# HKUST-Aerial-Robotics/VINS-Mobile

Hardware: AMD Instinct MI355X
Metric: VIO frames/sec (KLT+window solve), 640x480/150 feats/W=10 (higher is better)
Workload: dtype f64 (solve) / u8+i32+f32 (KLT)

## Files before the change

### vins-mobile_amd/abi.py

```python
import ctypes as C
import os

import numpy as np

VIO_OK = 0
VIO_EINVAL, VIO_ENODEV, VIO_ENOMEM, VIO_ECAP, VIO_ESTATE, VIO_ETIMEOUT = -1, -2, -3, -4, -5, -6
VIO_MAX_PRIOR_BLOCKS = 96
VIO_MAX_TRACE = 64
VIO_INIT_BA_MAX_FRAMES = 32
VIO_BLOCK_POSE, VIO_BLOCK_SPEEDBIAS, VIO_BLOCK_EXPOSE = 0, 1, 2
VIO_MARGIN_OLD, VIO_MARGIN_SECOND_NEW, VIO_MARGIN_NONE = 0, 1, 2
STAGES = ["setup_imu", "setup_prior", "eval_prior", "eval_imu", "eval_proj", "scale", "schur", "rhs", "cholesky",
          "tri_solve", "quad_form", "dogleg", "cost_eval", "new2old", "marg_build", "marg_chol", "total",
          "p_zero", "p_fact", "p_gram", "p_feat", "c_potrf", "c_trsm", "imu_raw", "c_wait", "q_w", "backsolve",
          "c_ahead", "tr_vec", "m_prior", "m_imu", "m_fact", "m_gram", "d0", "d1", "d2", "d3", "d4", "d5",
          "v_gd", "v_dot", "v_step", "v_plus", "v_gmax", "v_rest", "b_init", "b_pose", "b_asp", "b_band", "b_gn",
          "e_head", "e_copy", "e_h0dx", "e_tail", "x0", "x1", "x2", "x3", "s0", "s1", "s2", "s3"]

_dp = C.POINTER(C.c_double)
_ip = C.POINTER(C.c_int32)


class VioConfig(C.Structure):
    _fields_ = [
        ("window_size", C.c_int32), ("max_features", C.c_int32), ("max_factors", C.c_int32),
        ("max_iterations", C.c_int32), ("image_rows", C.c_int32), ("image_cols", C.c_int32),
        ("max_corners", C.c_int32), ("min_dist", C.c_int32), ("freq", C.c_int32),
        ("lk_win", C.c_int32), ("lk_levels", C.c_int32), ("lk_max_iters", C.c_int32),
        ("lk_eps", C.c_double), ("lk_min_eig", C.c_double), ("quality_level", C.c_double),
        ("f_threshold", C.c_double), ("f_confidence", C.c_double),
        ("fx", C.c_double), ("fy", C.c_double), ("cx", C.c_double), ("cy", C.c_double),
        ("gravity", C.c_double), ("acc_n", C.c_double), ("acc_w", C.c_double),
        ("gyr_n", C.c_double), ("gyr_w", C.c_double), ("cauchy_a", C.c_double),
    ]


def hip_runtime(lib=None):
    lib = lib or load_product()
    buf, n = C.create_string_buffer(4096), C.c_int32()
    lib.vio_hip_runtime(buf, 4096, C.byref(n))
    return [p for p in buf.value.decode().split(";") if p]


def host_pool_width():
    lib = load_product()
    n = C.c_int32(0)
    return int(lib.vio_host_pool_width(C.byref(n))), int(n.value)


def default_config(**kw):
    c = VioConfig(
        window_size=10, max_features=1000, max_factors=8192, max_iterations=10,
        image_rows=640, image_cols=480, max_corners=70, min_dist=30, freq=3,
        lk_win=21, lk_levels=3, lk_max_iters=30, lk_eps=0.01, lk_min_eig=1e-4,
        quality_level=0.01, f_threshold=1.0, f_confidence=0.99,
        fx=526.600, fy=526.678, cx=243.481, cy=315.280,
        gravity=9.805, acc_n=0.5, acc_w=0.002, gyr_n=0.2, gyr_w=4.0e-5, cauchy_a=1.0)
    for k, v in kw.items():
        setattr(c, k, v)
    return c


class VioPreintegration(C.Structure):
    _fields_ = [
        ("sum_dt", C.c_double), ("delta_p", C.c_double * 3), ("delta_q", C.c_double * 4),
        ("delta_v", C.c_double * 3), ("linearized_ba", C.c_double * 3),
        ("linearized_bg", C.c_double * 3), ("jacobian", C.c_double * 225),
        ("covariance", C.c_double * 225),
    ]


PREINT_DOUBLES = C.sizeof(VioPreintegration) // 8


class VioPrior(C.Structure):
    _fields_ = [
        ("n", C.c_int32), ("n_blocks", C.c_int32),
        ("block_kind", C.c_int32 * VIO_MAX_PRIOR_BLOCKS),
        ("block_index", C.c_int32 * VIO_MAX_PRIOR_BLOCKS),
        ("block_offset", C.c_int32 * VIO_MAX_PRIOR_BLOCKS),
        ("block_x0", _dp), ("linearized_jacobians", _dp), ("linearized_residuals", _dp),
    ]


class VioWindow(C.Structure):
    _fields_ = [
        ("window_size", C.c_int32), ("n_features", C.c_int32), ("n_factors", C.c_int32),
        ("marginalization_flag", C.c_int32),
        ("pose", _dp), ("speed_bias", _dp), ("ex_pose", _dp), ("inv_depth", _dp),
        ("factor_host", _ip), ("factor_target", _ip), ("factor_feature", _ip),
        ("factor_pts_i", _dp), ("factor_pts_j", _dp),
        ("preint", C.POINTER(VioPreintegration)), ("prior", C.POINTER(VioPrior)),
        ("loop_frame", C.c_int32), ("loop_pose", _dp),
        ("use_origin_override", C.c_int32), ("origin_yaw_deg", C.c_double),
        ("origin_p", C.c_double * 3),
        ("raw_pose", _dp), ("raw_speed_bias", _dp), ("raw_inv_depth", _dp),
        ("next_prior", C.POINTER(VioPrior)),
        ("resident_prior", C.c_int32),
    ]


class VioSolveStats(C.Structure):
    _fields_ = [
        ("initial_cost", C.c_double), ("final_cost", C.c_double),
        ("iterations", C.c_int32), ("termination", C.c_int32),
        ("num_successful_steps", C.c_int32), ("num_unsuccessful_steps", C.c_int32),
        ("it_cost", C.c_double * VIO_MAX_TRACE), ("it_radius", C.c_double * VIO_MAX_TRACE),
        ("it_step_norm", C.c_double * VIO_MAX_TRACE),
        ("it_relative_decrease", C.c_double * VIO_MAX_TRACE),
        ("it_gradient_max_norm", C.c_double * VIO_MAX_TRACE),
        ("it_flags", C.c_int32 * VIO_MAX_TRACE),
    ]


class VioObs(C.Structure):
    _fields_ = [("id", C.c_int32), ("x", C.c_double), ("y", C.c_double), ("z", C.c_double)]


class VioImuMsg(C.Structure):
    _fields_ = [("header", C.c_double), ("acc", C.c_double * 3), ("gyr", C.c_double * 3)]


class VioKeyframeData(C.Structure):
    _fields_ = [("header", C.c_double), ("translation", C.c_double * 3), ("rotation", C.c_double * 4)]


class VioPnpFeature(C.Structure):
    _fields_ = [("id", C.c_int32), ("observation", C.c_double * 2), ("position", C.c_double * 3), ("track_num", C.c_int32)]


class VioVinsResult(C.Structure):
    _fields_ = [("header", C.c_double), ("Ba", C.c_double * 3), ("Bg", C.c_double * 3), ("P", C.c_double * 3),
                ("R", C.c_double * 9), ("V", C.c_double * 3)]


class VioPnpWindow(C.Structure):
    _fields_ = [("n_frames", C.c_int32), ("pose", _dp), ("speed", _dp), ("bias", _dp), ("fixed", C.POINTER(C.c_uint8)),
                ("ex_pose", _dp), ("preint", C.POINTER(VioPreintegration)), ("feat_start", _ip), ("observation", _dp),
                ("position", _dp), ("track_num", _ip)]


class VioInitFrame(C.Structure):
    _fields_ = [("header", C.c_double), ("R", C.c_double * 9), ("T", C.c_double * 3), ("is_key_frame", C.c_int32),
                ("n_samples", C.c_int32), ("dt", _dp), ("acc", _dp), ("gyr", _dp), ("acc_0", C.c_double * 3),
                ("gyr_0", C.c_double * 3)]


class VioFrameResult(C.Structure):
    _fields_ = [("action", C.c_int32), ("error", C.c_int32), ("marginalization_flag", C.c_int32),
                ("failure_reasons", C.c_int32), ("track_num", C.c_int32), ("n_features", C.c_int32),
                ("n_factors", C.c_int32), ("n_loop_factors", C.c_int32), ("stats", VioSolveStats)]


class VioInitBaProblem(C.Structure):
    _fields_ = [("frame_num", C.c_int32), ("l", C.c_int32), ("n_points", C.c_int32), ("c_rotation", _dp), ("c_translation", _dp),
                ("points", _dp), ("point_ok", C.POINTER(C.c_uint8)), ("feat_start", _ip), ("obs_frame", _ip), ("obs_xy", _dp),
                ("ok", C.c_int32)]


class VioInitSfmProblem(C.Structure):
    _fields_ = [("frame_num", C.c_int32), ("l", C.c_int32), ("n_features", C.c_int32), ("feat_start", _ip), ("obs_frame", _ip),
                ("obs_xy", _dp), ("relative_mode", C.c_int32), ("R_hint", _dp), ("n_extra", C.c_int32), ("extra_guess", _ip),
                ("extra_start", _ip), ("extra_feature", _ip), ("extra_xy", _dp), ("status", C.c_int32), ("inliers", C.c_int32),
                ("relative_R", C.c_double * 9), ("relative_T", C.c_double * 3), ("q", _dp), ("T", _dp), ("points", _dp),
                ("point_ok", C.POINTER(C.c_uint8)), ("extra_R", _dp), ("extra_T", _dp)]


(VIO_INIT_SFM_OK, VIO_INIT_SFM_FAIL_RELATIVE, VIO_INIT_SFM_FAIL_CHAIN, VIO_INIT_SFM_FAIL_BA, VIO_INIT_SFM_FAIL_PNP) = range(5)


# ... 417 lines not shown
```

### vins-mobile_amd/csrc/marg_core.h

```cpp
#pragma once

#include "solver_core.h"

namespace vio {

struct MargOut {
  int *n;
  int *kind, *index, *offset;
  double *x0;
  double *J;
  double *r;
  double *scratch;
  int ncap;
};

template <class MP>
struct MargWorkT {
  MP Am;
  int ld;
  ldsd bm;
  ldsd tol;
  ldsd ldinv;
  ldsd hff, gf, einv;
  ldsd prdx, prr;
// ... 138 lines not shown
    const double y0 = rsq_cut(b[0], tol[0]);
    const double l10 = b[1] * y0, l20 = b[3] * y0, l30 = b[6] * y0;
    const double y1 = rsq_cut(fma(-l10, l10, b[2]), tol[1]);
    const double l21 = fma(-l20, l10, b[4]) * y1, l31 = fma(-l30, l10, b[7]) * y1;
    const double y2 = rsq_cut(fma(-l21, l21, fma(-l20, l20, b[5])), tol[2]);
    const double l32 = fma(-l31, l21, fma(-l30, l20, b[8])) * y2;
    const double y3 = rsq_cut(fma(-l32, l32, fma(-l31, l31, fma(-l30, l30, b[9]))), tol[3]);
    double M[10];
    M[0] = y0;
    M[1] = -(l10 * y0) * y1, M[2] = y1;
    M[3] = -fma(l21, M[1], l20 * y0) * y2, M[4] = -(l21 * M[2]) * y2, M[5] = y2;
    M[6] = -fma(l32, M[3], fma(l31, M[1], l30 * y0)) * y3, M[7] = -fma(l32, M[4], l31 * M[2]) * y3, M[8] = -(l32 * M[5]) * y3, M[9] = y3;
    double mop = 0.0;
#pragma unroll
    for (int q = 0; q < 10; q++) mop = mi == q ? M[q] : mop;
    const v4d z = {0.0, 0.0, 0.0, 0.0};
    const v4d V = mfma_f64(mop, A[cb], z), VE = mfma_f64(mop, E[cb], z);
    const double vv = V[0], ve = VE[0];
    A = mfma_f64(-vv, vv, A);
    E = mfma_f64(-vv, ve, E);
    keep[cb] = n >= 4 * cb + kq ? vv : ve;
    const double yn = (n & 3) == 0 ? y0 : (n & 3) == 1 ? y1 : (n & 3) == 2 ? y2 : y3;
    myinv = (n >> 2) == cb ? yn : myinv;
  }
  if (n < nvalid) {
#pragma unroll
    for (int j = 0; j < 4; j++) {
      const int c = kq + 4 * j;
      if (c < nvalid) D[n * ld + c] = keep[j];
    }
    if (kq == 0) ldinv_k[n] = myinv;
  }
}

template <class MP>
VIO_DEV void dtile_trsm(MP Aik, MP Dkk, cldsd ldinv_k, int ld, int rows, int lane) {
  const int n = lane & 15, kq = lane >> 4;
  double a[4];
  dtile_load_op(Aik, n * ld + kq, a);
  const v4d b = dtile_load_acc(Dkk, kq * ld + n, ld);
  const double dg = ldinv_k[n];
  v4d acc = {0.0, 0.0, 0.0, 0.0};
#pragma unroll
  for (int s4 = 0; s4 < 4; s4++) {
    const int kk = 4 * s4 + kq;
    const double bb = kk < n ? b[s4] : (kk == n ? dg : 0.0);
    acc = mfma_f64(a[s4], bb, acc);
  }
  dtile_store_acc(Aik, kq * ld + n, ld, acc, kq, rows);
}
template <class MP>
VIO_DEV void dtile_forward_diag(MP Dkk, cldsd ldinv_k, ldsd bk, int ld, int nvalid, int lane) {
  const int c = lane & 15;
  double s = ldinv_k[c] * bk[c];
#pragma unroll
  for (int n = 0; n < 15; n++) {
    const double x = Dkk[n * ld + c], bn = bk[n];
    s = fma(n < c ? x : 0.0, n < c ? bn : 0.0, s);
  }
  __builtin_amdgcn_wave_barrier();
  if (lane < 16 && c < nvalid) bk[c] = s;
}
template <class MP>
VIO_DEV void dtile_rhs_update(MP Lik, ldsd bi, cldsd yk, int ld, int rows, int lane) {
  const int r = lane >> 2, p = lane & 3;
  auto Lr = Lik + r * ld + p;
  double s = Lr[0] * yk[p];
  s = fma(Lr[4], yk[p + 4], s);
  s = fma(Lr[8], yk[p + 8], s);
  s = fma(Lr[12], yk[p + 12], s);
  s = quad_sum_f64(s);
  if (p == 0 && r < rows) bi[r] -= s;
}
template <class MP>
VIO_DEV void dtile_update2(MP C0, MP A0, MP B0, int rows0, int cols0, MP C1, MP A1, MP B1, int rows1, int cols1, int ld, int lane) {
  const int n = lane & 15, kq = lane >> 4, op = n * ld + kq, acc = kq * ld + n;
  double a0[4], b0[4], a1[4], b1[4];
  dtile_load_op(A0, op, a0), dtile_load_op(B0, op, b0), dtile_load_op(A1, op, a1), dtile_load_op(B1, op, b1);
  v4d c0 = dtile_load_acc(C0, acc, ld), c1 = dtile_load_acc(C1, acc, ld);
#pragma unroll
  for (int s4 = 0; s4 < 4; s4++) {
    c0 = mfma_f64(-a0[s4], b0[s4], c0);
    c1 = mfma_f64(-a1[s4], b1[s4], c1);
  }
  dtile_store_acc(C0, acc, ld, c0, kq, rows0, n < cols0);
  dtile_store_acc(C1, acc, ld, c1, kq, rows1, n < cols1);
}

template <class MP>
VIO_DEV void mtile_forward_diag(MP Dkk, cldsd ldinv_k, ldsd bk, int ld, int nvalid, int lane) {
  const int c = lane & 15;
  const bool cok = c < nvalid;
  double s = cok ? ldinv_k[c] * bk[c] : 0.0;
#pragma unroll
  for (int n = 0; n < 15; n++) {
    const bool in = cok && n < c;
    const double x = Dkk[(in ? n : 0) * ld + (in ? c : 0)], bn = bk[in ? n : 0];
    s = fma(in ? x : 0.0, bn, s);
  }
  __builtin_amdgcn_wave_barrier();
  if (lane < 16 && cok) bk[c] = s;
}
template <class MP>
VIO_DEV void mtile_rhs_update(MP Lik, ldsd bi, cldsd yk, int ld, int rows, int lane) {
  const int r = lane >> 2, p = lane & 3;
  const bool ok = r < rows;
  auto Lr = Lik + (ok ? r : 0) * ld + p;
  double s = Lr[0] * yk[p];
  s = fma(Lr[4], yk[p + 4], s);
  s = fma(Lr[8], yk[p + 8], s);
  s = fma(Lr[12], yk[p + 12], s);
  s = quad_sum_f64(s);
  if (p == 0 && ok) bi[r] -= s;
}

template <class MW>
VIO_DEV void marg_cholesky_tiles(const Ctx &cx, MW &m, int pos) {
  const int nt = (pos + 15) >> 4;
  const int tid_ = VIO_TID(cx), wave = __builtin_amdgcn_readfirstlane(tid_ >> 6), nw = cx.nt >> 6, lane = tid_ & 63;
  const int li = lane & 15, kq = lane >> 4;
  auto tile = [&](int ti, int tj) { return m.Am + tri_off(ti) + 16 * tj; };
  auto rows_of = [&](int ti) { return pos - 16 * ti < 16 ? pos - 16 * ti : 16; };
  auto tol_of = [&](int ti) {
    const int j = 16 * ti + (lane & 15);
    const double t = m.tol[j];
    return j < pos ? t : 1.0;
  };
  if (wave == 0) potrf16_cut_wave(tile(0, 0), tile(0, 0), tri_ld(0), rows_of(0), false, tol_of(0), m.ldinv, lane);
  VIO_SYNC();
  for (int k = 0; k < nt; k++) {
    const int ntb = nt - k - 1;
    for (int bi = wave; bi < ntb; bi += nw)
      tile_trsm(tile(k + 1 + bi, k), tri_ld(k + 1 + bi), rows_of(k + 1 + bi), tile(k, k), tri_ld(k), m.ldinv + 16 * k, li, kq);
    if (wave == nw - 1) mtile_forward_diag(tile(k, k), m.ldinv + 16 * k, m.bm + 16 * k, tri_ld(k), rows_of(k), lane);
    VIO_SYNC();
    if (wave == 0) {
      if (ntb > 0) potrf16_cut_wave(tile(k + 1, k + 1), tile(k + 1, k), tri_ld(k + 1), rows_of(k + 1), true, tol_of(k + 1), m.ldinv + 16 * (k + 1), lane);
    } else {
      const int stride = nw - 1;
      for (int bi = wave - 1; bi < ntb; bi += stride)
        mtile_rhs_update(tile(k + 1 + bi, k), m.bm + 16 * (k + 1 + bi), m.bm + 16 * k, tri_ld(k + 1 + bi), rows_of(k + 1 + bi), lane);
      const int npairs = ntb * (ntb + 1) / 2;
      for (int pr = wave; pr < npairs; pr += stride) {
        int a = 0;
        while ((a + 1) * (a + 2) / 2 <= pr) a++;
        const int i0 = k + 1 + a, j0 = k + 1 + pr - a * (a + 1) / 2;
        tile_update(tile(i0, j0), tri_ld(i0), rows_of(i0), tile(i0, k), tile(j0, k), tri_ld(j0), rows_of(j0), li, kq);
      }
    }
    VIO_SYNC();
  }
}

template <int PASS = -1, class MW>
VIO_DEV void marginalize_window_impl(const Ctx &cx, const WinView &v, cldsd xpose, cldsd xsb, cldsd xfeat, cldsd ex,
                                     MW &m, const MargOut &out) {
  const int W = v.W, P = v.P, F = v.F;
  const int flag = v.marg_flag;
  const bool wide = PASS < 0 ? m.wide : PASS == 1;
  const int pn = v.prior_n;
  bool run = (flag == 0);
  if (flag == 1) {
    bool touches = false;
    for (int b = 0; b < v.prior_nb; b++)
      if (v.pr_kind[b] == 0 && v.pr_index[b] == W - 1) touches = true;
    run = pn > 0 && touches;
  }
  if (!run) {
    if (cx.tid == 0) out.n[0] = -1, out.n[1] = 0, out.n[2] = 0, out.n[3] = 0;
    return;
  }
  if (cx.tid == 0) {
    for (int i = 0; i <= P; i++) m.col_pose[i] = -1;
    for (int i = 0; i < P; i++) m.col_sb[i] = -1;
    m.col_ex[0] = -1;
    for (int b = 0; b < v.prior_nb; b++) {
      int kind = v.pr_kind[b], idx = v.pr_index[b];
      if (kind == 0) m.col_pose[idx] = -2;
      else if (kind == 1) m.col_sb[idx] = -2;
      else m.col_ex[0] = -2;
    }
    if (flag == 0) m.col_pose[0] = m.col_sb[0] = m.col_pose[1] = m.col_sb[1] = -2;
  }
  VIO_SYNC();
  if (flag == 0) {
    VIO_PARFOR(p, v.npairs)
      if (v.pair_h[p] == 0 && v.pair_t[p] != P) m.col_pose[v.pair_t[p]] = -2, m.col_ex[0] = -2;
  }
  VIO_SYNC();
  if (cx.tid == 0) {
    int pos = 0, nblocks = 0;
    if (flag == 0) {
      m.col_pose[0] = pos, pos += 6;
      m.col_sb[0] = pos, pos += 9;
    } else {
      m.col_pose[W - 1] = pos, pos += 6;
    }
    const int mdrop = pos;
    auto keep = [&](int kind, int idx, int col, int new_index) {
      out.kind[nblocks] = kind, out.index[nblocks] = new_index, out.offset[nblocks] = col - mdrop;
      double *x0 = out.x0 + 9 * nblocks;
      for (int q = 0; q < 9; q++) x0[q] = 0.0;
      cldsd src = kind == 0 ? xpose + 7 * idx : kind == 1 ? xsb + 9 * idx : ex;
      int gs = kind == 1 ? 9 : 7;
      for (int q = 0; q < gs; q++) x0[q] = src[q];
      nblocks++;
    };
    for (int i = 0; i < P; i++)
      if (m.col_pose[i] == -2) {
        m.col_pose[i] = pos;
        keep(0, i, pos, flag == 0 ? i - 1 : (i == W ? W - 1 : i));
        pos += 6;
      }
    for (int i = 0; i < P; i++)
      if (m.col_sb[i] == -2) {
        m.col_sb[i] = pos;
        keep(1, i, pos, flag == 0 ? i - 1 : (i == W ? W - 1 : i));
        pos += 9;
      }
    if (m.col_ex[0] == -2) {
      m.col_ex[0] = pos;
      keep(2, 0, pos, 0);
      pos += 6;
    }
    m.meta[0] = pos, m.meta[1] = mdrop, m.meta[2] = pos - mdrop, m.meta[3] = nblocks;
  }
  VIO_SYNC();
  const int pos = m.meta[0], mdrop = m.meta[1], n = m.meta[2], nblocks = m.meta[3];
  const int ld = m.ld;
  if (pos > ld || n > out.ncap) {
    if (cx.tid == 0) out.n[0] = -2, out.n[1] = 0, out.n[2] = mdrop, out.n[3] = pos;
    return;
  }
  VIO_PARFOR(q, (int)tri_doubles(pos)) m.Am[q] = 0.0;
  VIO_PARFOR(q, pos) m.bm[q] = 0.0;
  VIO_PARFOR(f, F) m.hff[f] = 0.0, m.gf[f] = 0.0;
  if (flag == 0) VIO_PARFOR(q, 12 * F) {
    const int f = q / 12, c = q - 12 * f;
    v.WTf[(size_t)f * v.n6cap + (c < 6 ? c : 6 * P + c - 6)] = 0.0;
  }
  VIO_SYNC();
  if (pn > 0) {
    VIO_PARFOR(b, v.prior_nb) {
      int kind = v.pr_kind[b], idx = v.pr_index[b], o = v.pr_offset[b];
      const double *x0 = v.pr_x0 + 9 * b;
      int base = kind == 0 ? m.col_pose[idx] : kind == 1 ? m.col_sb[idx] : m.col_ex[0];
      int ls = kind == 1 ? 9 : 6;
      for (int k = 0; k < ls; k++) m.pcol[o + k] = base + k;
      if (kind == 0) prior_block_dx(7, xpose + 7 * idx, x0, m.prdx + o);
      else if (kind == 1) prior_block_dx(9, xsb + 9 * idx, x0, m.prdx + o);
      else prior_block_dx(7, ex, x0, m.prdx + o);
    }
    VIO_PARFOR(i, pn) m.prr[i] = v.prb0[i];
    VIO_SYNC();
    dense_matvec_cols(cx, v.prH0, pn, m.prdx, [&](int i, double sacc) { VIO_ATOMIC_ADD(m.prr + i, sacc); });
    {
      constexpr int kU = 12;
      const int nst = (pn + kU - 1) / kU;
      VIO_PARFOR(q, pn * nst) {
        const int a = q / nst, b0 = kU * (q - a * nst);
        const int ca = m.pcol[a];
        double x[kU];
#pragma unroll
        for (int u = 0; u < kU; u++) x[u] = v.prH0[a * pn + (b0 + u < pn ? b0 + u : b0)];
        VIO_SCHED_FENCE();
#pragma unroll
        for (int u = 0; u < kU; u++) {
          if (b0 + u >= pn) continue;
          const int cb = m.pcol[b0 + u];
          if (ca >= cb) m.Am[tri_at(ca, cb)] = x[u];
        }
      }
    }
    VIO_SYNC();
    VIO_PARFOR(a, pn) m.bm[m.pcol[a]] += m.prr[a];
    VIO_SYNC();
  }
  stamp(cx, ST_M_PRIOR);
  if (flag == 0) {
    if (!wide) {
      const int i = (int)cx.nt - 1 - VIO_TID(cx);
      if (i <= P) {
        double R[9];
        if (i == P) qtoR(Quat{ex[3], ex[4], ex[5], ex[6]}, R);
        else qtoR(Quat{xpose[7 * i + 3], xpose[7 * i + 4], xpose[7 * i + 5], xpose[7 * i + 6]}, R);
        for (int k = 0; k < 9; k++) m.rot[9 * i + k] = R[k];
      }
    }
    if (cx.tid == 0)
      imu_eval_raw(v.gravity, v.preint, xpose, xsb, xpose + 7, xsb + 9, v.imu_r, v.imu_J);
    VIO_SYNC();
    VIO_PARFOR(r, 15) {
      const double *info = v.imu_info + r * 15;
      double s = 0;
      for (int k = 0; k < 15; k++) s += info[k] * v.imu_r[k];
      v.imu_Mr[r] = s;
    }
    VIO_PARFOR(q, 450) {
      int r = q / 30, c = q % 30;
      const double *info = v.imu_info + r * 15;
      double s = 0;
      for (int k = 0; k < 15; k++) s += info[k] * v.imu_J[k * 30 + c];
      v.imu_M[q] = s;
    }
    VIO_SYNC();
    VIO_PARFOR(q, 900) {
      int a = q / 30, b = q % 30;
      int ca = a < 6 ? m.col_pose[0] + a : a < 15 ? m.col_sb[0] + a - 6 : a < 21 ? m.col_pose[1] + a - 15 : m.col_sb[1] + a - 21;
      int cb = b < 6 ? m.col_pose[0] + b : b < 15 ? m.col_sb[0] + b - 6 : b < 21 ? m.col_pose[1] + b - 15 : m.col_sb[1] + b - 21;
      double s = 0;
      for (int k = 0; k < 15; k++) s += v.imu_J[k * 30 + a] * v.imu_M[k * 30 + b];
      if (ca >= cb) VIO_ATOMIC_ADD(m.Am + tri_at(ca, cb), s);
    }
    VIO_PARFOR(a, 30) {
      int ca = a < 6 ? m.col_pose[0] + a : a < 15 ? m.col_sb[0] + a - 6 : a < 21 ? m.col_pose[1] + a - 15 : m.col_sb[1] + a - 21;
      double s = 0;
      for (int k = 0; k < 15; k++) s += v.imu_J[k * 30 + a] * v.imu_Mr[k];
      VIO_ATOMIC_ADD(m.bm + ca, s);
    }
    stamp(cx, ST_M_IMU);
    auto add_lower = [&](int ra, int ca, double val) {
      if (ra >= ca) VIO_ATOMIC_ADD(m.Am + tri_at(ra, ca), val);
      else VIO_ATOMIC_ADD(m.Am + tri_at(ca, ra), val);
    };
    if (wide) {
      const double cc = 1.0 / v.cauchy_b;
      int S0 = 0, nb0 = 0;
      for (int p = 0; p < v.npairs && v.pair_h[p] == 0; p++)
        if (v.pair_t[p] != P) S0 = (v.pair_s1[p] + 1) & ~1, nb0 = p + 1;
      auto G = m.stage;
      const int CH = m.stage_slots;
      if (CH < 2) {
        if (cx.tid == 0) out.n[0] = -3, out.n[1] = 0;
        return;
      }
      const int lane_d = VIO_TID(cx) & 63;
      const bool dv = lane_d < nb0;
      const int d_s0 = dv ? v.pair_s0[lane_d] : 0, d_s1 = dv ? v.pair_s1[lane_d] : 0;
      const int d_t = dv ? ((v.pair_h[lane_d] != 0 || v.pair_t[lane_d] == P) ? -1 : v.pair_t[lane_d]) : -1;
      for (int c0 = 0; c0 < S0; c0 += CH) {
        VIO_PARFOR(slot, (S0 - c0 < CH ? S0 - c0 : CH)) {
          const int rec = v.srec_i[c0 + slot];
          double pij[6];
  #pragma unroll
          for (int c = 0; c < 6; c++) pij[c] = v.srec_d[6 * (size_t)(c0 + slot) + c];
          if (rec < 0) continue;
          const int t = (rec >> 8) & 255, f = rec >> 16;
          if ((rec & 255) != 0 || t == P) continue;
          double r[2], Ji[12], Jj[12], Jex[12], Jl[2];
          projection_eval(v.s_info, xpose, xpose + 7 * t, ex, xfeat[f], pij, pij + 3, true, r, Ji, Jj, Jex, Jl);
          double sq = r[0] * r[0] + r[1] * r[1];
          double sr = sqrt(1.0 / (1.0 + sq * cc));
          auto g = G + slot * kWideSlot; auto gx = g + kWideStride;
  #pragma unroll
          for (int rr = 0; rr < 2; rr++) {
  #pragma unroll
            for (int c = 0; c < 6; c++) {
              g[rr * kWideRow + c] = Ji[rr * 6 + c] * sr, g[rr * kWideRow + 6 + c] = Jj[rr * 6 + c] * sr;
              gx[rr * kWideRowX + c] = Jex[rr * 6 + c] * sr;
            }
            g[rr * kWideRow + 12] = r[rr] * sr, g[rr * kWideRow + 13] = Jl[rr] * sr;
          }
          const double s2 = sr * sr;
          double *wf = v.WTf + (size_t)f * v.n6cap;
  #pragma unroll
          for (int c = 0; c < 6; c++) {
            wf[6 * t + c] = (Jj[c] * Jl[0] + Jj[6 + c] * Jl[1]) * s2;
            VIO_ATOMIC_ADD(wf + c, (Ji[c] * Jl[0] + Ji[6 + c] * Jl[1]) * s2);
            VIO_ATOMIC_ADD(wf + 6 * P + c, (Jex[c] * Jl[0] + Jex[6 + c] * Jl[1]) * s2);
          }
          VIO_ATOMIC_ADD(m.hff + f, (Jl[0] * Jl[0] + Jl[1] * Jl[1]) * s2);
          VIO_ATOMIC_ADD(m.gf + f, (Jl[0] * r[0] + Jl[1] * r[1]) * s2);
        }
        VIO_SYNC();
        stamp(cx, ST_M_FACT);
        auto flush1 = [&](int t, int row, int col, double val) {
          const int c0p = m.col_pose[0], ctp = m.col_pose[t];
          if (row < 6) {
            if (col <= row) VIO_ATOMIC_ADD(m.Am + tri_at(c0p + row, c0p + col), val);
          } else if (row < 12) {
            if (col < 6) add_lower(ctp + row - 6, c0p + col, val);
            else if (col < 12 && col <= row) VIO_ATOMIC_ADD(m.Am + tri_at(ctp + row - 6, ctp + col - 6), val);
          } else if (row == 12) {
            if (col < 6) VIO_ATOMIC_ADD(m.bm + c0p + col, val);
            else if (col < 12) VIO_ATOMIC_ADD(m.bm + ctp + col - 6, val);
          }
        };
        auto flush2 = [&](int t, int row, int col, double val) {
          if (row >= 6) return;
          const int cx0 = m.col_ex[0];
          if (col < 6) add_lower(cx0 + row, m.col_pose[0] + col, val);
          else if (col < 12) add_lower(cx0 + row, m.col_pose[t] + col - 6, val);
          else if (col == 12) VIO_ATOMIC_ADD(m.bm + cx0 + row, val);
        };
        auto flush3 = [&](int row, int col, double val) {
          if (row < 6 && col <= row) VIO_ATOMIC_ADD(m.Am + tri_at(m.col_ex[0] + row, m.col_ex[0] + col), val);
        };
        {
          const int tid_ = VIO_TID(cx), wave = __builtin_amdgcn_readfirstlane(tid_ >> 6), nw = cx.nt >> 6, lane = tid_ & 63;
          const int li = lane & 15, kq = lane >> 4;
          for (int p = wave; p < nb0 && p < 64; p += nw) {
            const int b_s0 = __builtin_amdgcn_readlane(d_s0, p), b_s1 = __builtin_amdgcn_readlane(d_s1, p);
            const int t = __builtin_amdgcn_readlane(d_t, p);
            if (t < 0) continue;
            const int s_lo = b_s0 > c0 ? b_s0 : c0, s_hi = b_s1 < c0 + CH ? b_s1 : c0 + CH;
            if (s_lo >= s_hi) continue;
            v4d a1 = {0.0, 0.0, 0.0, 0.0}, a2 = a1, a3 = a1;
            const bool lv = li < kWideRow, lx = li < kWideRowX;
            const int go = (s_lo - c0 + (kq >> 1)) * kWideSlot + (kq & 1) * kWideRow + (lv ? li : 0);
            const int gxo = (s_lo - c0 + (kq >> 1)) * kWideSlot + kWideStride + (kq & 1) * kWideRowX + (lx ? li : 0);
            const int nsteps = (s_hi - s_lo + 1) >> 1;
            constexpr int kB = 6;
            for (int st0 = 0; st0 < nsteps; st0 += kB) {
              double av[kB], xv[kB];
  #pragma unroll
              for (int j = 0; j < kB; j++) {
                const bool in = st0 + j < nsteps && s_lo + 2 * (st0 + j) + (kq >> 1) < s_hi;
                av[j] = G[in ? go + 2 * (st0 + j) * kWideSlot : 0], xv[j] = G[in ? gxo + 2 * (st0 + j) * kWideSlot : 0];
              }
              VIO_SCHED_FENCE();
  #pragma unroll
              for (int j = 0; j < kB; j++) {
                const bool in = st0 + j < nsteps && s_lo + 2 * (st0 + j) + (kq >> 1) < s_hi;
                const double a = (lv && in) ? av[j] : 0.0, x = (lx && in) ? xv[j] : 0.0;
                if (st0 + j < nsteps) a1 = mfma_f64(a, a, a1), a2 = mfma_f64(x, a, a2), a3 = mfma_f64(x, x, a3);
              }
            }
  #pragma unroll
            for (int r4 = 0; r4 < 4; r4++) {
              flush1(t, kq + 4 * r4, li, a1[r4]), flush2(t, kq + 4 * r4, li, a2[r4]), flush3(kq + 4 * r4, li, a3[r4]);
            }
          }
        }
        VIO_SYNC();
        stamp(cx, ST_M_GRAM);
      }
    } else {
      const double cc = 1.0 / v.cauchy_b;
      int S0 = 0, nb0 = 0;
      for (int p = 0; p < v.npairs && v.pair_h[p] == 0; p++)
        if (v.pair_t[p] != P) S0 = (v.pair_s1[p] + 1) & ~1, nb0 = p + 1;
      auto G = m.stage;
      const int CH = m.stage_slots;
      if (CH < 2) {
        if (cx.tid == 0) out.n[0] = -3, out.n[1] = 0;
        return;
      }
      const int lane_d = VIO_TID(cx) & 63;
      const bool dv = lane_d < nb0;
      const int d_s0 = dv ? v.pair_s0[lane_d] : 0, d_s1 = dv ? v.pair_s1[lane_d] : 0;
      const int d_t = dv ? ((v.pair_h[lane_d] != 0 || v.pair_t[lane_d] == P) ? -1 : v.pair_t[lane_d]) : -1;
      const bool one_pass = CH <= (int)cx.nt;
      int rec_n = -1;
      double pij_n[6] = {0, 0, 0, 0, 0, 0};
      if (one_pass) {
        const int sl0 = VIO_TID(cx);
        if (sl0 < S0 && sl0 < CH) {
          rec_n = v.srec_i[sl0];
  #pragma unroll
          for (int c = 0; c < 6; c++) pij_n[c] = v.srec_d[6 * (size_t)sl0 + c];
        }
      }
      auto flush = [&](const v4d &acc, int ctp) {
        const int lane_f = VIO_TID(cx) & 63, li = lane_f & 15, kq = lane_f >> 4;
        const int c0p = m.col_pose[0], cx0 = m.col_ex[0];
        auto image = [](int a, int k, int &blk, int &off, int &neg) {
          neg = 0;
          if (a < 3) return blk = k, off = a, neg = k, true;
          if (k != 0 || a == 9) return false;
          if (a < 6) return blk = 0, off = a, true;
          if (a < 9) return blk = 1, off = a - 3, true;
          return blk = 2, off = a - 10, true;
// ... 185 lines not shown
```

### vins-mobile_amd/csrc/spmd.h

```cpp
#pragma once

#include <math.h>
#include <stdint.h>

#include "vio_math.h"

#if defined(VIO_EMUL) || defined(VIO_SIMT)
#define VIO_HOST_BUILD 1
#endif
#ifdef VIO_HOST_BUILD
#define VIO_DEV inline
#define VIO_ATOMIC_ADD(p, v) ::vio::atomic_add((p), (v))
#else
#define VIO_DEV __device__ __forceinline__
#define VIO_ATOMIC_ADD(p, v) ::vio::atomic_add((p), (v))
#endif
#if defined(VIO_EMUL)
#define VIO_SYNC() ((void)0)
#define VIO_SYNC_LDS() ((void)0)
#elif defined(VIO_SIMT)
#define VIO_SYNC() __syncthreads()
#define VIO_SYNC_LDS() __syncthreads()
#else
#define VIO_SYNC() __syncthreads()
#define VIO_SYNC_LDS()                                                      \
  do {                                                                      \
    __builtin_amdgcn_fence(__ATOMIC_RELEASE, "workgroup", "local");         \
    __builtin_amdgcn_s_barrier();                                           \
    __builtin_amdgcn_fence(__ATOMIC_ACQUIRE, "workgroup", "local");         \
  } while (0)
#endif
#ifdef VIO_HOST_BUILD
#define VIO_TID(cx) ((int)(cx).tid)
#else
#define VIO_TID(cx) ::vio::hw_tid((cx).wave64)
#endif
#define VIO_PARFOR(i, n) for (int i = VIO_TID(cx); i < (int)(n); i += (int)cx.nt)
#ifdef VIO_HOST_BUILD
#define VIO_OPAQUE(x) (x)
#else
#define VIO_OPAQUE(x) ::vio::opaque_tid(x)
#endif

#ifdef VIO_HOST_BUILD
#define VIO_AS3
#else
#define VIO_AS3 __attribute__((address_space(3)))
#endif

namespace vio {

#ifndef VIO_HOST_BUILD
__device__ __forceinline__ int opaque_tid(int t) {
  asm volatile("" : "+v"(t));
  return t;
}
__device__ __forceinline__ int hw_tid(int wave64) {
  int t;
  asm volatile("v_mbcnt_lo_u32_b32 %0, -1, %1\n\tv_mbcnt_hi_u32_b32 %0, -1, %0" : "=v"(t) : "s"(wave64));
  return t;
}
#endif

typedef VIO_AS3 double *ldsd;
typedef const VIO_AS3 double *cldsd;
typedef VIO_AS3 int *ldsi;

#ifdef VIO_HOST_BUILD
inline void atomic_add(double *p, double v) { *p += v; }
inline void atomic_add_noret(double *p, double v) { *p += v; }
#else
__device__ __forceinline__ void atomic_add_noret(double *p, double v) {
  (void)__hip_atomic_fetch_add(p, v, __ATOMIC_RELAXED, __HIP_MEMORY_SCOPE_AGENT);
}
__device__ __forceinline__ void atomic_add(ldsd p, double v) {
  __hip_atomic_fetch_add(p, v, __ATOMIC_RELAXED, __HIP_MEMORY_SCOPE_WORKGROUP);
}
__device__ __forceinline__ void atomic_add(double *p, double v) {
  __hip_atomic_fetch_add(p, v, __ATOMIC_RELAXED, __HIP_MEMORY_SCOPE_WORKGROUP);
}
#endif

enum Stage {
  ST_SETUP_IMU = 0, ST_SETUP_PRIOR, ST_EVAL_PRIOR, ST_EVAL_IMU, ST_EVAL_PROJ, ST_SCALE, ST_SCHUR, ST_RHS, ST_CHOL,
  ST_TRISOLVE, ST_QUADFORM, ST_DOGLEG, ST_COST_EVAL, ST_NEW2OLD, ST_MARG_BUILD, ST_MARG_CHOL, ST_TOTAL,
  ST_P_ZERO, ST_P_FACT, ST_P_GRAM, ST_P_FEAT,
  ST_C_POTRF, ST_C_TRSM,
  ST_IMU_RAW,
  ST_C_WAIT, ST_Q_W, ST_BACKSOLVE, ST_C_AHEAD,
  ST_TR_VEC,
  ST_M_PRIOR, ST_M_IMU, ST_M_FACT, ST_M_GRAM,
  ST_D0, ST_D1, ST_D2, ST_D3, ST_D4, ST_D5,
  ST_V_GD,
  ST_V_DOT, ST_V_STEP,
  ST_V_PLUS,
  ST_V_GMAX,
  ST_V_REST,
  ST_B_INIT, ST_B_POSE, ST_B_ASP, ST_B_BAND, ST_B_GN,
  ST_E_HEAD, ST_E_COPY, ST_E_H0DX, ST_E_TAIL,
  ST_X0, ST_X1, ST_X2, ST_X3,
  ST_S0, ST_S1, ST_S2, ST_S3,
  ST_COUNT = 64
};

struct Ctx {
  int tid, nt;
  int wave64 = 0;
  ldsd red;
  mutable int red_phase = 0;
  long long *prof;
  int wrot = 0;
  int prof_tid = 0;
  VIO_AS3 long long *lprof;
  int coop = 1, member = 0;
  unsigned coop_spin = 1u << 24;
  mutable unsigned coop_seq = 0;
};

VIO_DEV void stamp(const Ctx &cx, int stage) {
#if !defined(VIO_EMUL)
  if (cx.prof && cx.tid == cx.prof_tid) {
    long long t = clock64();
    cx.lprof[stage] += t - cx.lprof[ST_COUNT - 1];
    cx.lprof[ST_COUNT - 1] = t;
  }
#else
  (void)cx, (void)stage;
#endif
}

#ifndef VIO_EMUL
template <int CTRL, int ROWMASK>
__device__ __forceinline__ double dpp_move_f64(double v) {
  int lo = __builtin_amdgcn_update_dpp(0, __double2loint(v), CTRL, ROWMASK, 0xf, false);
  int hi = __builtin_amdgcn_update_dpp(0, __double2hiint(v), CTRL, ROWMASK, 0xf, false);
  return __hiloint2double(hi, lo);
}
__device__ __forceinline__ double wave_sum_f64(double v) {
  v += dpp_move_f64<0x111, 0xf>(v);
  v += dpp_move_f64<0x112, 0xf>(v);
  v += dpp_move_f64<0x114, 0xf>(v);
  v += dpp_move_f64<0x118, 0xf>(v);
  v += dpp_move_f64<0x142, 0xa>(v);
  v += dpp_move_f64<0x143, 0xc>(v);
  return __hiloint2double(__builtin_amdgcn_readlane(__double2hiint(v), 63), __builtin_amdgcn_readlane(__double2loint(v), 63));
}
__device__ __forceinline__ double wave_max_f64(double v) {
  v = fmax(v, dpp_move_f64<0x111, 0xf>(v));
  v = fmax(v, dpp_move_f64<0x112, 0xf>(v));
  v = fmax(v, dpp_move_f64<0x114, 0xf>(v));
  v = fmax(v, dpp_move_f64<0x118, 0xf>(v));
  v = fmax(v, dpp_move_f64<0x142, 0xa>(v));
  v = fmax(v, dpp_move_f64<0x143, 0xc>(v));
  return __hiloint2double(__builtin_amdgcn_readlane(__double2hiint(v), 63), __builtin_amdgcn_readlane(__double2loint(v), 63));
}
#endif
VIO_DEV double block_sum(const Ctx &cx, double v) {
#ifdef VIO_EMUL
  return v;
#else
  const int nw = cx.nt >> 6;
  ldsd red = cx.red + (cx.red_phase ^= 1) * 3 * nw;
  v = wave_sum_f64(v);
  if ((cx.tid & 63) == 0) red[cx.tid >> 6] = v;
  VIO_SYNC();
  double s = 0;
  for (int w = 0; w < nw; w++) s += red[w];
  return s;
#endif
}
VIO_DEV void block_sum3(const Ctx &cx, double &a, double &b, double &c) {
#ifndef VIO_EMUL
  const int nw = cx.nt >> 6;
  ldsd red = cx.red + (cx.red_phase ^= 1) * 3 * nw;
  a = wave_sum_f64(a), b = wave_sum_f64(b), c = wave_sum_f64(c);
  if ((cx.tid & 63) == 0) red[cx.tid >> 6] = a, red[nw + (cx.tid >> 6)] = b, red[2 * nw + (cx.tid >> 6)] = c;
  VIO_SYNC();
  a = b = c = 0;
  for (int w = 0; w < nw; w++) a += red[w], b += red[nw + w], c += red[2 * nw + w];
#else
  (void)cx, (void)a, (void)b, (void)c;
#endif
}
VIO_DEV double block_max(const Ctx &cx, double v) {
#ifdef VIO_EMUL
  return v;
#else
  const int nw = cx.nt >> 6;
  ldsd red = cx.red + (cx.red_phase ^= 1) * 3 * nw;
  v = wave_max_f64(v);
  if ((cx.tid & 63) == 0) red[cx.tid >> 6] = v;
  VIO_SYNC();
  double s = red[0];
  for (int w = 1; w < nw; w++) s = fmax(s, red[w]);
  return s;
#endif
}

#if defined(VIO_HOST_BUILD)
#define VIO_PRIO(n) ((void)0)
#else
#define VIO_PRIO(n) __builtin_amdgcn_s_setprio(n)
#endif
#if defined(VIO_HOST_BUILD)
#define VIO_FLAG_STORE(p, x) (*(volatile int *)(p) = (x))
#define VIO_FLAG_LOAD(p) (*(volatile int *)(p))
#else
#define VIO_FLAG_STORE(p, x) __hip_atomic_store((p), (x), __ATOMIC_RELAXED, __HIP_MEMORY_SCOPE_WORKGROUP)
#define VIO_FLAG_LOAD(p) __hip_atomic_load((p), __ATOMIC_RELAXED, __HIP_MEMORY_SCOPE_WORKGROUP)
#endif
#if defined(VIO_HOST_BUILD)
#define VIO_SCHED_FENCE() ((void)0)
#else
#define VIO_SCHED_FENCE() __builtin_amdgcn_sched_barrier(0)
#endif

}
```

Before: 199,900.

## Add wave-level LDS marginalization front end and MFMA IMU gram for narrow path

Splits the marginalization front end into a general path (kept for the wide case) and a new LDS path. The new path computes column assignments with wave ballots and popcounts instead of serial thread-0 loops. It overlaps the zeroing, rotation and IMU raw evaluation across different waves and prefetches prior-H0 strips into registers so the matvec and scatter happen in one pass. The IMU information-weighted Jacobian gram is computed with f64 MFMA on a single wave instead of several PARFOR passes separated by barriers. The aim is to cut block-wide syncs and serial work, at the cost of much more complex code with limits (2P+1<=64) and more register pressure.

```diff
diff --git a/vins-mobile_amd/abi.py b/vins-mobile_amd/abi.py
--- a/vins-mobile_amd/abi.py
+++ b/vins-mobile_amd/abi.py
@@ -15,7 +15,7 @@
           "p_zero", "p_fact", "p_gram", "p_feat", "c_potrf", "c_trsm", "imu_raw", "c_wait", "q_w", "backsolve",
           "c_ahead", "tr_vec", "m_prior", "m_imu", "m_fact", "m_gram", "d0", "d1", "d2", "d3", "d4", "d5",
           "v_gd", "v_dot", "v_step", "v_plus", "v_gmax", "v_rest", "b_init", "b_pose", "b_asp", "b_band", "b_gn",
-          "e_head", "e_copy", "e_h0dx", "e_tail", "x0", "x1", "x2", "x3", "s0", "s1", "s2", "s3"]
+          "e_head", "e_copy", "e_h0dx", "e_tail", "x0", "x1", "x2", "x3", "s0", "s1", "s2", "s3", "mt_raw"]
 
 _dp = C.POINTER(C.c_double)
 _ip = C.POINTER(C.c_int32)
diff --git a/vins-mobile_amd/csrc/marg_core.h b/vins-mobile_amd/csrc/marg_core.h
--- a/vins-mobile_amd/csrc/marg_core.h
+++ b/vins-mobile_amd/csrc/marg_core.h
@@ -314,12 +314,10 @@
   }
 }
 
-template <int PASS = -1, class MW>
-VIO_DEV void marginalize_window_impl(const Ctx &cx, const WinView &v, cldsd xpose, cldsd xsb, cldsd xfeat, cldsd ex,
-                                     MW &m, const MargOut &out) {
+template <class MW>
+VIO_DEV bool marg_front_general(const Ctx &cx, const WinView &v, cldsd xpose, cldsd xsb, cldsd ex, MW &m, const MargOut &out, int dims[4]) {
   const int W = v.W, P = v.P, F = v.F;
   const int flag = v.marg_flag;
-  const bool wide = PASS < 0 ? m.wide : PASS == 1;
   const int pn = v.prior_n;
   bool run = (flag == 0);
   if (flag == 1) {
@@ -330,7 +328,7 @@
   }
   if (!run) {
     if (cx.tid == 0) out.n[0] = -1, out.n[1] = 0, out.n[2] = 0, out.n[3] = 0;
-    return;
+    return false;
   }
   if (cx.tid == 0) {
     for (int i = 0; i <= P; i++) m.col_pose[i] = -1;
@@ -350,6 +348,7 @@
       if (v.pair_h[p] == 0 && v.pair_t[p] != P) m.col_pose[v.pair_t[p]] = -2, m.col_ex[0] = -2;
   }
   VIO_SYNC();
+  stamp(cx, ST_MT_HEAD);
   if (cx.tid == 0) {
     int pos = 0, nblocks = 0;
     if (flag == 0) {
@@ -388,11 +387,12 @@
     m.meta[0] = pos, m.meta[1] = mdrop, m.meta[2] = pos - mdrop, m.meta[3] = nblocks;
   }
   VIO_SYNC();
+  stamp(cx, ST_MT_COLS);
   const int pos = m.meta[0], mdrop = m.meta[1], n = m.meta[2], nblocks = m.meta[3];
   const int ld = m.ld;
   if (pos > ld || n > out.ncap) {
     if (cx.tid == 0) out.n[0] = -2, out.n[1] = 0, out.n[2] = mdrop, out.n[3] = pos;
-    return;
+    return false;
   }
   VIO_PARFOR(q, (int)tri_doubles(pos)) m.Am[q] = 0.0;
   VIO_PARFOR(q, pos) m.bm[q] = 0.0;
@@ -402,6 +402,7 @@
     v.WTf[(size_t)f * v.n6cap + (c < 6 ? c : 6 * P + c - 6)] = 0.0;
   }
   VIO_SYNC();
+  stamp(cx, ST_MT_ZERO);
   if (pn > 0) {
     VIO_PARFOR(b, v.prior_nb) {
       int kind = v.pr_kind[b], idx = v.pr_index[b], o = v.pr_offset[b];
@@ -415,7 +416,9 @@
     }
     VIO_PARFOR(i, pn) m.prr[i] = v.prb0[i];
     VIO_SYNC();
+    stamp(cx, ST_MT_DX);
     dense_matvec_cols(cx, v.prH0, pn, m.prdx, [&](int i, double sacc) { VIO_ATOMIC_ADD(m.prr + i, sacc); });
+    stamp(cx, ST_MT_H0DX);
     {
       constexpr int kU = 12;
       const int nst = (pn + kU - 1) / kU;
@@ -438,48 +441,308 @@
     VIO_PARFOR(a, pn) m.bm[m.pcol[a]] += m.prr[a];
     VIO_SYNC();
   }
+  dims[0] = pos, dims[1] = mdrop, dims[2] = n, dims[3] = nblocks;
+  return true;
+}
+
+template <class MW>
+VIO_DEV bool marg_front_lds(const Ctx &cx, const WinView &v, cldsd xpose, cldsd xsb, cldsd ex, MW &m, const MargOut &out, int dims[4]) {
+  const int W = v.W, P = v.P, F = v.F;
+  const int flag = v.marg_flag;
+  const int pn = v.prior_n, nb = v.prior_nb;
+  const int tid_ = VIO_TID(cx), nt_ = (int)cx.nt, wave = __builtin_amdgcn_readfirstlane(tid_ >> 6), nw = nt_ >> 6, lane = tid_ & 63;
+  if ((flag != 0 && flag != 1) || 2 * P + 1 > 64) {
+    if (cx.tid == 0) out.n[0] = 2 * P + 1 > 64 ? -3 : -1, out.n[1] = 0, out.n[2] = 0, out.n[3] = 0;
+    return false;
+  }
+  const bool hv = lane < nb;
+  int hk = -1, hi = 0, ho = 0;
+  double hx[9] = {0, 0, 0, 0, 0, 0, 0, 0, 0};
+  if (hv) {
+    hk = v.pr_kind[lane], hi = v.pr_index[lane], ho = v.pr_offset[lane];
+#pragma unroll
+    for (int q = 0; q < 9; q++) hx[q] = v.pr_x0[9 * lane + q];
+  }
+  int tv[2] = {-1, -1};
+#pragma unroll
+  for (int r = 0; r < 2; r++) {
+    const int p = 64 * r + lane;
+    if (flag == 0 && p < v.npairs) {
+      const int h = v.pair_h[p], t = v.pair_t[p];
+      tv[r] = (h == 0 && t != P) ? t : -1;
+    }
+  }
+  constexpr int kStrip = 25;
+  int nparts = pn > 0 ? nt_ / pn : 1;
+  const int need = (pn + 4 * kStrip - 1) / (4 * kStrip);
+  nparts = nparts < need ? need : (nparts > 8 ? 8 : nparts);
+  const int per = pn > 0 ? (pn + nparts - 1) / nparts : 0;
+  const bool one_strip = pn > 0 && pn * nparts <= nt_ && per <= kStrip;
+  const int hpart = tid_ / (pn > 0 ? pn : 1), hc = tid_ - hpart * pn, hk0 = hpart * per;
+  const int hnb = (one_strip && tid_ < pn * nparts) ? (hk0 + per < pn ? per : pn - hk0) : 0;
+  double hs[kStrip];
+#pragma unroll
+  for (int j = 0; j < kStrip; j++) hs[j] = 0.0;
+  if (hnb > 0) {
+    const double *hp = v.prH0 + (size_t)hk0 * pn + hc;
+#pragma unroll
+    for (int j = 0; j < kStrip; j++) hs[j] = hp[(size_t)(j < hnb ? j : 0) * pn];
+  }
+  VIO_SCHED_FENCE();
+  if (wave == 0) {
+    hk = lane < nb ? hk : -1;
+    const bool cand = lane <= 2 * P;
+    const int jk = lane < P ? 0 : lane < 2 * P ? 1 : 2, ji = lane < P ? lane : lane < 2 * P ? lane - P : 0;
+    bool inv = false;
+    for (int b0 = 0; b0 < nb; b0 += 64) {
+      int k = hk, i = hi;
+      if (b0 > 0) {
+        const int b = b0 + lane;
+        k = b < nb ? v.pr_kind[b] : -1, i = b < nb ? v.pr_index[b] : 0;
+      }
+      const int cnt = nb - b0 < 64 ? nb - b0 : 64;
+      for (int q = 0; q < cnt; q++) {
+        const int kq = __builtin_amdgcn_readlane(k, q), iq = __builtin_amdgcn_readlane(i, q);
+        inv = inv || (kq == jk && (kq == 2 || iq == ji));
+      }
+    }
+    unsigned pmask = 0;
+    for (int p0 = 0; p0 < v.npairs && flag == 0; p0 += 64) {
+      int t = p0 == 0 ? tv[0] : tv[1];
+      if (p0 >= 128) {
+        const int p = p0 + lane;
+        const bool ok = p < v.npairs;
+        const int h = v.pair_h[ok ? p : 0], t2 = v.pair_t[ok ? p : 0];
+        t = (ok && h == 0 && t2 != P) ? t2 : -1;
+      }
+      for (int tt = 0; tt < P; tt++)
+        if (__builtin_amdgcn_ballot_w64(t == tt) != 0) pmask |= 1u << tt;
+    }
+    if (jk == 0) inv = inv || ((pmask >> ji) & 1u) != 0 || (flag == 0 && ji < 2);
+    else if (jk == 1) inv = inv || (flag == 0 && ji < 2);
+    else inv = inv || pmask != 0;
+    stamp(cx, ST_MT_HEAD);
+    const bool touch = __builtin_amdgcn_ballot_w64(cand && jk == 0 && ji == W - 1 && inv) != 0;
+    const bool run = flag == 0 || (pn > 0 && touch);
+    const bool drop = flag == 0 ? (jk < 2 && ji == 0) : (jk == 0 && ji == W - 1);
+    const bool kept = cand && inv && !drop;
+    const unsigned long long km = __builtin_amdgcn_ballot_w64(kept), below = km & ((1ull << lane) - 1ull);
+    const unsigned long long pm = (1ull << P) - 1ull, sm = pm << P;
+    const int mdrop = flag == 0 ? 15 : 6;
+    const int mypos = mdrop + 6 * __builtin_popcountll(below & pm) + 9 * __builtin_popcountll(below & sm), myb = __builtin_popcountll(below);
+    const int pos = mdrop + 6 * __builtin_popcountll(km & pm) + 9 * __builtin_popcountll(km & sm) + 6 * (int)((km >> (2 * P)) & 1ull);
+    if (cand) {
+      const int col = drop ? (jk == 1 ? 6 : 0) : kept ? mypos : -1;
+      if (jk == 0) m.col_pose[ji] = col;
+      else if (jk == 1) m.col_sb[ji] = col;
+      else m.col_ex[0] = col, m.col_pose[P] = -1;
+    }
+    if (lane == 0) m.meta[0] = run ? pos : -1, m.meta[1] = mdrop, m.meta[2] = pos - mdrop, m.meta[3] = __builtin_popcountll(km);
+    if (run && kept) {
+      out.kind[myb] = jk, out.index[myb] = jk == 2 ? 0 : flag == 0 ? ji - 1 : (ji == W ? W - 1 : ji), out.offset[myb] = mypos - mdrop;
+      cldsd src = jk == 0 ? xpose + 7 * ji : jk == 1 ? xsb + 9 * ji : ex;
+      const int gs = jk == 1 ? 9 : 7;
+      double x0[9];
+#pragma unroll
+      for (int q = 0; q < 9; q++) x0[q] = src[q < gs ? q : 0];
+#pragma unroll
+      for (int q = 0; q < 9; q++) out.x0[9 * myb + q] = q < gs ? x0[q] : 0.0;
+    }
+    stamp(cx, ST_MT_COLS);
+    __builtin_amdgcn_wave_barrier();
+    if (run && pn > 0)
+      for (int b0 = 0; b0 < nb; b0 += 64) {
+        const int b = b0 + lane;
+        if (b >= nb) continue;
+        int k = hk, i = hi, o = ho;
+        if (b0 > 0) {
+          k = v.pr_kind[b], i = v.pr_index[b], o = v.pr_offset[b];
+#pragma unroll
+          for (int q = 0; q < 9; q++) hx[q] = v.pr_x0[9 * b + q];
+        }
+        const int base = k == 0 ? m.col_pose[i] : k == 1 ? m.col_sb[i] : m.col_ex[0];
+        const int ls = k == 1 ? 9 : 6;
+        for (int kk = 0; kk < ls; kk++) m.pcol[o + kk] = base + kk;
+        if (k == 0) prior_block_dx(7, xpose + 7 * i, hx, m.prdx + o);
+        else if (k == 1) prior_block_dx(9, xsb + 9 * i, hx, m.prdx + o);
+        else prior_block_dx(7, ex, hx, m.prdx + o);
+      }
+    stamp(cx, ST_MT_DX);
+  }
+  {
+    const int z0 = nw > 1 ? tid_ - 64 : tid_, zn = nw > 1 ? nt_ - 64 : nt_;
+    if (z0 >= 0) {
+      for (int i = z0; i < pn; i += zn) m.prr[i] = v.prb0[i];
+      const int nam = (int)tri_doubles(m.ld);
+      for (int q = z0; q < nam; q += zn) m.Am[q] = 0.0;
+      for (int q = z0; q < m.ld; q += zn) m.bm[q] = 0.0;
+      for (int f = z0; f < F; f += zn) m.hff[f] = 0.0, m.gf[f] = 0.0;
+      if (flag == 0)
+        for (int q = z0; q < 12 * F; q += zn) {
+          const int f = q / 12, c = q - 12 * f;
+          v.WTf[(size_t)f * v.n6cap + (c < 6 ? c : 6 * P + c - 6)] = 0.0;
+        }
+    }
+  }
+  if (flag == 0) {
+    const int i = nt_ - 1 - tid_;
+    if (i <= P) {
+      double R[9];
+      if (i == P) qtoR(Quat{ex[3], ex[4], ex[5], ex[6]}, R);
+      else qtoR(Quat{xpose[7 * i + 3], xpose[7 * i + 4], xpose[7 * i + 5], xpose[7 * i + 6]}, R);
+      for (int k = 0; k < 9; k++) m.rot[9 * i + k] = R[k];
+    } else if (i == P + 1) {
+      imu_eval_raw(v.gravity, v.preint, xpose, xsb, xpose + 7, xsb + 9, v.imu_r, v.imu_J);
+    }
+  }
+  VIO_SYNC_LDS();
+  stamp(cx, ST_MT_ZERO);
+  const int pos = m.meta[0], mdrop = m.meta[1], n = m.meta[2];
+  if (pos < 0) {
+    if (cx.tid == 0) out.n[0] = -1, out.n[1] = 0, out.n[2] = 0, out.n[3] = 0;
+    return false;
+  }
+  if (pos > m.ld || n > out.ncap) {
+    if (cx.tid == 0) out.n[0] = -2, out.n[1] = 0, out.n[2] = mdrop, out.n[3] = pos;
+    return false;
+  }
+  if (pn > 0) {
+    if (one_strip) {
+      if (hnb > 0) {
+        const int cc = m.pcol[hc];
+        double sacc = 0;
+#pragma unroll
+        for (int j = 0; j < kStrip; j++) {
+          const int k = hk0 + (j < hnb ? j : 0);
+          sacc += (j < hnb ? hs[j] : 0.0) * m.prdx[k];
+          const int ck = m.pcol[k];
+          if (j < hnb && ck >= cc) m.Am[tri_at(ck, cc)] = hs[j];
+        }
+        VIO_ATOMIC_ADD(m.prr + hc, sacc);
+      }
+    } else {
+      dense_matvec_cols(cx, v.prH0, pn, m.prdx, [&](int i, double sacc) { VIO_ATOMIC_ADD(m.prr + i, sacc); });
+      constexpr int kU = 12;
+      const int nst = (pn + kU - 1) / kU;
+      VIO_PARFOR(q, pn * nst) {
+        const int a = q / nst, b0 = kU * (q - a * nst);
+        const int ca = m.pcol[a];
+        double x[kU];
+#pragma unroll
+        for (int u = 0; u < kU; u++) x[u] = v.prH0[a * pn + (b0 + u < pn ? b0 + u : b0)];
+        VIO_SCHED_FENCE();
+#pragma unroll
+        for (int u = 0; u < kU; u++) {
+          if (b0 + u >= pn) continue;
+          const int cb = m.pcol[b0 + u];
+          if (ca >= cb) m.Am[tri_at(ca, cb)] = x[u];
+        }
+      }
+    }
+  }
+  VIO_SYNC();
+  stamp(cx, ST_MT_H0DX);
+  dims[0] = pos, dims[1] = mdrop, dims[2] = n, dims[3] = m.meta[3];
+  return true;
+}
+
+template <class MW>
+VIO_DEV void marg_imu_general(const Ctx &cx, const WinView &v, cldsd xpose, cldsd xsb, MW &m) {
+  if (cx.tid == 0)
+    imu_eval_raw(v.gravity, v.preint, xpose, xsb, xpose + 7, xsb + 9, v.imu_r, v.imu_J);
+  VIO_SYNC();
+  stamp(cx, ST_MT_RAW);
+  VIO_PARFOR(r, 15) {
+    const double *info = v.imu_info + r * 15;
+    double s = 0;
+    for (int k = 0; k < 15; k++) s += info[k] * v.imu_r[k];
+    v.imu_Mr[r] = s;
+  }
+  VIO_PARFOR(q, 450) {
+    int r = q / 30, c = q % 30;
+    const double *info = v.imu_info + r * 15;
+    double s = 0;
+    for (int k = 0; k < 15; k++) s += info[k] * v.imu_J[k * 30 + c];
+    v.imu_M[q] = s;
+  }
+  VIO_SYNC();
+  VIO_PARFOR(q, 900) {
+    int a = q / 30, b = q % 30;
+    int ca = a < 6 ? m.col_pose[0] + a : a < 15 ? m.col_sb[0] + a - 6 : a < 21 ? m.col_pose[1] + a - 15 : m.col_sb[1] + a - 21;
+    int cb = b < 6 ? m.col_pose[0] + b : b < 15 ? m.col_sb[0] + b - 6 : b < 21 ? m.col_pose[1] + b - 15 : m.col_sb[1] + b - 21;
+    double s = 0;
+    for (int k = 0; k < 15; k++) s += v.imu_J[k * 30 + a] * v.imu_M[k * 30 + b];
+    if (ca >= cb) VIO_ATOMIC_ADD(m.Am + tri_at(ca, cb), s);
+  }
+  VIO_PARFOR(a, 30) {
+    int ca = a < 6 ? m.col_pose[0] + a : a < 15 ? m.col_sb[0] + a - 6 : a < 21 ? m.col_pose[1] + a - 15 : m.col_sb[1] + a - 21;
+    double s = 0;
+    for (int k = 0; k < 15; k++) s += v.imu_J[k * 30 + a] * v.imu_Mr[k];
+    VIO_ATOMIC_ADD(m.bm + ca, s);
+  }
+}
+
+template <class MW>
+VIO_DEV void marg_imu_lds(const Ctx &cx, const WinView &v, MW &m) {
+  const int tid_ = VIO_TID(cx), wave = __builtin_amdgcn_readfirstlane(tid_ >> 6), nw = cx.nt >> 6, lane = tid_ & 63;
+  if (wave != ((nw - cx.wrot) & (nw - 1))) return;
+  const int nn = lane & 15, kq = lane >> 4;
+  double a4[4], b0[4], b1[4];
+#pragma unroll
+  for (int s4 = 0; s4 < 4; s4++) {
+    const int k = 4 * s4 + kq, kc = k < 15 ? k : 0;
+    a4[s4] = v.imu_info[(nn < 15 ? nn : 0) * 15 + kc];
+    b0[s4] = v.imu_J[kc * 30 + nn];
+    b1[s4] = nn == 14 ? v.imu_r[kc] : v.imu_J[kc * 30 + 16 + (nn < 14 ? nn : 0)];
+  }
+  VIO_SCHED_FENCE();
+  v4d T0 = {0, 0, 0, 0}, T1 = {0, 0, 0, 0};
+#pragma unroll
+  for (int s4 = 0; s4 < 4; s4++) {
+    const bool kok = 4 * s4 + kq < 15;
+    a4[s4] = (kok && nn < 15) ? a4[s4] : 0.0, b0[s4] = kok ? b0[s4] : 0.0, b1[s4] = (kok && nn < 15) ? b1[s4] : 0.0;
+    T0 = mfma_f64(a4[s4], b0[s4], T0), T1 = mfma_f64(a4[s4], b1[s4], T1);
+  }
+  v4d G00 = {0, 0, 0, 0}, G10 = {0, 0, 0, 0}, G11 = {0, 0, 0, 0};
+#pragma unroll
+  for (int s4 = 0; s4 < 4; s4++) {
+    G00 = mfma_f64(b0[s4], T0[s4], G00);
+    G10 = mfma_f64(b1[s4], T0[s4], G10);
+    G11 = mfma_f64(b1[s4], T1[s4], G11);
+  }
+  auto lc = [&](int a) {
+    return a < 6 ? m.col_pose[0] + a : a < 15 ? m.col_sb[0] + a - 6 : a < 21 ? m.col_pose[1] + a - 15 : m.col_sb[1] + a - 21;
+  };
+  const int cn = lc(nn), cn1 = lc(16 + (nn < 14 ? nn : 0));
+#pragma unroll
+  for (int r4 = 0; r4 < 4; r4++) {
+    const int row = kq + 4 * r4, R = 16 + row;
+    if (row >= nn) VIO_ATOMIC_ADD(m.Am + tri_at(lc(row), cn), G00[r4]);
+    if (R < 30) {
+      VIO_ATOMIC_ADD(m.Am + tri_at(lc(R), cn), G10[r4]);
+      if (nn < 14 && R >= 16 + nn) VIO_ATOMIC_ADD(m.Am + tri_at(lc(R), cn1), G11[r4]);
+    } else if (R == 30) {
+      VIO_ATOMIC_ADD(m.bm + cn, G10[r4]);
+      if (nn < 14) VIO_ATOMIC_ADD(m.bm + cn1, G11[r4]);
+    }
+  }
+}
+
+template <int PASS = -1, class MW>
+VIO_DEV void marginalize_window_impl(const Ctx &cx, const WinView &v, cldsd xpose, cldsd xsb, cldsd xfeat, cldsd ex,
+                                     MW &m, const MargOut &out) {
+  const int P = v.P, F = v.F;
+  const int flag = v.marg_flag;
+  const bool wide = PASS < 0 ? m.wide : PASS == 1;
+  const int pn = v.prior_n;
+  int dims[4];
+  if (wide ? !marg_front_general(cx, v, xpose, xsb, ex, m, out, dims) : !marg_front_lds(cx, v, xpose, xsb, ex, m, out, dims)) return;
+  const int pos = dims[0], mdrop = dims[1], n = dims[2], nblocks = dims[3];
+  if (!wide && pn > 0) VIO_PARFOR(a, pn) VIO_ATOMIC_ADD(m.bm + m.pcol[a], m.prr[a]);
   stamp(cx, ST_M_PRIOR);
   if (flag == 0) {
-    if (!wide) {
-      const int i = (int)cx.nt - 1 - VIO_TID(cx);
-      if (i <= P) {
-        double R[9];
-        if (i == P) qtoR(Quat{ex[3], ex[4], ex[5], ex[6]}, R);
-        else qtoR(Quat{xpose[7 * i + 3], xpose[7 * i + 4], xpose[7 * i + 5], xpose[7 * i + 6]}, R);
-        for (int k = 0; k < 9; k++) m.rot[9 * i + k] = R[k];
-      }
-    }
-    if (cx.tid == 0)
-      imu_eval_raw(v.gravity, v.preint, xpose, xsb, xpose + 7, xsb + 9, v.imu_r, v.imu_J);
-    VIO_SYNC();
-    VIO_PARFOR(r, 15) {
-      const double *info = v.imu_info + r * 15;
-      double s = 0;
-      for (int k = 0; k < 15; k++) s += info[k] * v.imu_r[k];
-      v.imu_Mr[r] = s;
-    }
-    VIO_PARFOR(q, 450) {
-      int r = q / 30, c = q % 30;
-      const double *info = v.imu_info + r * 15;
-      double s = 0;
-      for (int k = 0; k < 15; k++) s += info[k] * v.imu_J[k * 30 + c];
-      v.imu_M[q] = s;
-    }
-    VIO_SYNC();
-    VIO_PARFOR(q, 900) {
-      int a = q / 30, b = q % 30;
-      int ca = a < 6 ? m.col_pose[0] + a : a < 15 ? m.col_sb[0] + a - 6 : a < 21 ? m.col_pose[1] + a - 15 : m.col_sb[1] + a - 21;
-      int cb = b < 6 ? m.col_pose[0] + b : b < 15 ? m.col_sb[0] + b - 6 : b < 21 ? m.col_pose[1] + b - 15 : m.col_sb[1] + b - 21;
-      double s = 0;
-      for (int k = 0; k < 15; k++) s += v.imu_J[k * 30 + a] * v.imu_M[k * 30 + b];
-      if (ca >= cb) VIO_ATOMIC_ADD(m.Am + tri_at(ca, cb), s);
-    }
-    VIO_PARFOR(a, 30) {
-      int ca = a < 6 ? m.col_pose[0] + a : a < 15 ? m.col_sb[0] + a - 6 : a < 21 ? m.col_pose[1] + a - 15 : m.col_sb[1] + a - 21;
-      double s = 0;
-      for (int k = 0; k < 15; k++) s += v.imu_J[k * 30 + a] * v.imu_Mr[k];
-      VIO_ATOMIC_ADD(m.bm + ca, s);
-    }
+    if (wide) marg_imu_general(cx, v, xpose, xsb, m);
+    else marg_imu_lds(cx, v, m);
     stamp(cx, ST_M_IMU);
     auto add_lower = [&](int ra, int ca, double val) {
       if (ra >= ca) VIO_ATOMIC_ADD(m.Am + tri_at(ra, ca), val);
diff --git a/vins-mobile_amd/csrc/spmd.h b/vins-mobile_amd/csrc/spmd.h
--- a/vins-mobile_amd/csrc/spmd.h
+++ b/vins-mobile_amd/csrc/spmd.h
@@ -100,8 +100,11 @@
   ST_E_HEAD, ST_E_COPY, ST_E_H0DX, ST_E_TAIL,
   ST_X0, ST_X1, ST_X2, ST_X3,
   ST_S0, ST_S1, ST_S2, ST_S3,
+  ST_MT_RAW,
+  ST_MT_HEAD = ST_E_COPY, ST_MT_COLS = ST_E_H0DX, ST_MT_ZERO = ST_E_TAIL, ST_MT_DX = ST_B_ASP, ST_MT_H0DX = ST_B_GN,
   ST_COUNT = 64
 };
+static_assert(ST_MT_RAW < ST_COUNT - 1, "the stage slots are full");
 
 struct Ctx {
   int tid, nt;
```

New measurement: 201,500 (median of 6 runs). No clear change (+0.8%).
